# QZ1-boy/CDFO

Measured on NVIDIA B200. Metric: HR frames/sec, 1080p x4 LD-QP37, higher is better.
Workload: dtype bf16

## Files before the change

cdfo_b200/_lib.py:

```python
import ctypes
import os
import re
import weakref

import torch

_HERE = os.path.dirname(os.path.abspath(__file__))
SO_PATH = os.path.join(_HERE, "libcdfo_b200.so")

OK = 0
F32, F16, BF16 = 0, 1, 2
_DTYPES = {torch.float32: F32, torch.float16: F16, torch.bfloat16: BF16}


class CdfoError(RuntimeError):
    pass


_lib = None
HEADER = os.path.join(os.path.dirname(_HERE), "include", "cdfo_b200.h")


def _ctype(decl):
    d = decl.strip()
# ... 27 lines not shown
        fn.restype, fn.argtypes = res, args


def lib():
    global _lib
    if _lib is None:
        if not os.path.isfile(SO_PATH):
            raise CdfoError(
                "cdfo_b200: %s not found -- build it with `python cdfo_b200/csrc/build.py` "
                "(there is no CPU or PyTorch fallback for this path)" % SO_PATH)
        _lib = ctypes.CDLL(SO_PATH)
        _bind_prototypes(_lib)
    return _lib


_LAUNCHES = {"cdfo_mv_end_fix": 3, "cdfo_lra_fwd": 5, "cdfo_lra_c8_fwd": 5, "cdfo_mdta_fwd": 3, "cdfo_mdta_c8_fwd": 3, "cdfo_psnr_ssim_u8": 3,
             "cdfo_lra_mask_logits_fwd": 2,
             "cdfo_spatial_gate_c8_fwd": 2}
launch_count = 0


def call(name, *args):
    global launch_count
    rc = getattr(lib(), name)(*args)
    if rc != OK:
        check(rc, name)
    launch_count += _LAUNCHES.get(name, 1)
    return rc


def check(rc, what=""):
# ... 45 lines not shown
```

cdfo_b200/config.py:

```python
import os

tensor_core = True

dcn_gather = "tex"

conv_pair = os.environ.get("CDFO_CONV_PAIR", "1") != "0"

conv_fold_half = os.environ.get("CDFO_CONV_FOLD_HALF", "1") != "0"

conv_parity_planes = os.environ.get("CDFO_CONV_PARITY_PLANES", "1") != "0"
trunk_fused_resample = os.environ.get("CDFO_TRUNK_FUSED_RESAMPLE", "1") != "0"

head_dual = os.environ.get("CDFO_HEAD_DUAL", "1") != "0"

fused_head_dcn = os.environ.get("CDFO_FUSED_HEAD_DCN", "1") != "0"

features_c8 = os.environ.get("CDFO_FEATURES_C8", "1") != "0"
mdta_c8 = os.environ.get("CDFO_MDTA_C8", "1") != "0"
trunk_compose_1x1 = os.environ.get("CDFO_TRUNK_COMPOSE_1X1", "1") != "0"
trunk_fused_upsample = os.environ.get("CDFO_TRUNK_FUSED_UPSAMPLE", "1") != "0"
lra_logits_from_prior = os.environ.get("CDFO_LRA_LOGITS_FROM_PRIOR", "1") != "0"
```

cdfo_b200/csrc/cdfo_common.cuh:

```cuda
#pragma once
#include <cuda_bf16.h>
#include <cuda_fp16.h>
#include <cuda_runtime.h>
#include <stdarg.h>
#include <stdint.h>
#include <stdio.h>

#include "../../include/cdfo_b200.h"

namespace cdfo {

char *last_error_buf();
int fail(int code, const char *fmt, ...);

inline int check_launch(const char *what) {
  cudaError_t e = cudaGetLastError();
  if (e != cudaSuccess) return fail(CDFO_ERR_CUDA, "%s: %s", what, cudaGetErrorString(e));
  return CDFO_OK;
}

constexpr int kNumSMs = 148;

__host__ __device__ inline int ceil_div(int a, int b) { return (a + b - 1) / b; }
inline long long ceil_div_ll(long long a, long long b) { return (a + b - 1) / b; }
// ... 16 lines not shown
  const float v = __fadd_rn((float)pos, flow);
  const float g = __fsub_rn(__fdiv_rn(__fmul_rn(2.0f, v), (float)max(size - 1, 1)), 1.0f);
  return __fmul_rn(__fdiv_rn(__fadd_rn(g, 1.0f), 2.0f), (float)(size - 1));
}

struct LraTables {
  const float *kw;
  const float *kh;
  const float *k1;
  const float *r;
  float beta, bh;
};
int lra_col_sm100_launch(const float *vrow_t, const uint8_t *midx, const float *qsel, float *long_out, const LraTables &t, int B, int H, int W,
                         cudaStream_t s);

int pointwise_conv(const float *in1, const float *in2, const float *w, const float *bias, const float *resid1, const float *resid2,
                   float *out, int B, int K, int Co, int HW, int act, int mode, cudaStream_t s, void *out_c8 = nullptr,
                   int out_channels = 0, int channel0 = 0);

int conv3x3_pack_weight_raw(const float *w, void *out, int Cout, int Cin, int NT, int n_tiles, int streamed, int taps, cudaStream_t s);

}

#define CDFO_REQUIRE(cond, code, ...)                 \
  do {                                                \
    if (!(cond)) return cdfo::fail(code, __VA_ARGS__); \
  } while (0)
```

cdfo_b200/csrc/lra.cu:

```cuda
#include <cuda.h>
#include <cstring>

#include "cdfo_common.cuh"
#include "sm100_ptx.cuh"

namespace cdfo {

__device__ __forceinline__ float warp_max(float v) {
#pragma unroll
  for (int o = 16; o > 0; o >>= 1) v = fmaxf(v, __shfl_xor_sync(0xffffffffu, v, o));
  return v;
}
__device__ __forceinline__ float warp_sum(float v) {
#pragma unroll
  for (int o = 16; o > 0; o >>= 1) v += __shfl_xor_sync(0xffffffffu, v, o);
  return v;
}

__global__ void lra_mask_kernel(const float *__restrict__ u, const float *__restrict__ vmax, const float *__restrict__ qv,
                                uint8_t *__restrict__ midx, float *__restrict__ qsel, int HW) {
  __shared__ float vm[64];
  const int b = blockIdx.y;
  if (threadIdx.x < 64) vm[threadIdx.x] = vmax[b * 64 + threadIdx.x];
  __syncthreads();
// ... 836 lines not shown
  g_lra_col_tc = on != 0;
  return CDFO_OK;
}
extern "C" int cdfo_lra_set_win_tensor_core(int on) {
  g_lra_win_tc = on != 0;
  return CDFO_OK;
}

extern "C" size_t cdfo_lra_workspace_bytes(int B, int H, int W) {
  const size_t P = (size_t)B * H * W;
  return P * (1 + 4) + 3 * P * 64 * 4 + 256;
}

static int lra_run(const float *qv, const float *u, const float *vmax, const float *x, const float *x2, const float *tables,
                   float beta, float bh, const float *fuse_w, const float *fuse_b, float *out, void *out_c8, int out_channels,
                   int channel0, void *workspace, int B, int H, int W, void *stream);

extern "C" int cdfo_lra_fwd(const float *qv, const float *u, const float *vmax, const float *x, const float *x2, const float *tables,
                            float beta, float bh, const float *fuse_w, const float *fuse_b, float *out, void *workspace, int B,
                            int H, int W, void *stream) {
  return lra_run(qv, u, vmax, x, x2, tables, beta, bh, fuse_w, fuse_b, out, nullptr, 0, 0, workspace, B, H, W, stream);
}

extern "C" int cdfo_lra_c8_fwd(const float *qv, const float *u, const float *vmax, const float *x, const float *x2, const float *tables,
                               float beta, float bh, const float *fuse_w, const float *fuse_b, void *out_c8, int out_channels,
                               int channel0, void *workspace, int B, int H, int W, void *stream) {
  CDFO_REQUIRE(out_c8 && ((uintptr_t)out_c8 & 15) == 0, CDFO_ERR_NULL, "cdfo_lra_c8_fwd: out_c8 must be a 16-byte aligned pointer");
  CDFO_REQUIRE(out_channels % 8 == 0 && channel0 % 8 == 0 && channel0 >= 0 && channel0 + 64 <= out_channels, CDFO_ERR_SHAPE,
               "cdfo_lra_c8_fwd: channels [%d, %d) do not fit %d output channels (multiples of 8)", channel0, channel0 + 64, out_channels);
  return lra_run(qv, u, vmax, x, x2, tables, beta, bh, fuse_w, fuse_b, nullptr, out_c8, out_channels, channel0, workspace, B, H, W, stream);
}

static int lra_run(const float *qv, const float *u, const float *vmax, const float *x, const float *x2, const float *tables,
                   float beta, float bh, const float *fuse_w, const float *fuse_b, float *out, void *out_c8, int out_channels,
                   int channel0, void *workspace, int B, int H, int W, void *stream) {
  CDFO_REQUIRE(qv && u && vmax && x && tables && fuse_w && fuse_b && (out || out_c8) && workspace, CDFO_ERR_NULL, "cdfo_lra_fwd: NULL pointer");
  CDFO_REQUIRE(B > 0 && B <= 65535 && H > 0 && W > 0 && H % 8 == 0 && W % 8 == 0, CDFO_ERR_SHAPE,
               "cdfo_lra_fwd: H and W must be multiples of the window size 8 (got %d x %d)", H, W);
  cudaStream_t s = (cudaStream_t)stream;
  const size_t P = (size_t)B * H * W;
  const int HW = H * W;
  uint8_t *ws = (uint8_t *)workspace;
  float *qsel = (float *)ws;
  float *vrow_t = qsel + P;
  float *long_out = vrow_t + P * 64;
  float *loc_out = long_out + P * 64;
  uint8_t *midx = (uint8_t *)(loc_out + P * 64);
  LraTables t{tables, tables + 9, tables + 18, tables + 82, beta, bh};

  lra_mask_kernel<<<dim3(ceil_div(HW, 128), B), 128, 0, s>>>(u, vmax, qv, midx, qsel, HW);
// ... 42 lines not shown
  int col_done = 0;
  if (!g_lra_col_tf32 && g_lra_col_tc) {
    col_done = lra_col_sm100_launch(vrow_t, midx, qsel, long_out, t, B, H, W, s);
    if (col_done < 0) return col_done;
  }
  if (col_done) {
  } else if (g_lra_col_tf32) {
    lra_col_kernel<<<dim3(W, B), kColThreads, col_smem, s>>>(vrow_t, midx, qsel, long_out, t, H, W);
  } else {
    const size_t col16_smem = ((size_t)Hk * kQw + 64 * ((size_t)Hk / 2 + 4) + 2 * (size_t)(H + 8) + 16) * 4;
    lra_col_bf16_kernel<<<dim3(W, B), kColThreads, col16_smem, s>>>(vrow_t, midx, qsel, long_out, t, H, W);
  }
  if (g_lra_win_tc) lra_win_tc_kernel<<<dim3(W / 8, H / 8, B), kWinTcThreads, 0, s>>>(qv, midx, loc_out, H, W);
  else lra_win_kernel<<<dim3(W / 8, H / 8, B), kWinThreads, win_smem, s>>>(qv, midx, loc_out, H, W);
  if (int rc = check_launch("cdfo_lra_fwd")) return rc;
  return pointwise_conv(long_out, loc_out, fuse_w, fuse_b, x, x2, out, B, 128, 64, HW, 0, 1, s, out_c8, out_channels, channel0);
}
```

cdfo_b200/csrc/pointwise.cu:

```cuda
#include "cdfo_common.cuh"

namespace cdfo {
namespace pw {

constexpr int kTP = 64, kThreads = 256;
constexpr int kLdT = 72;

__device__ __forceinline__ uint32_t to_tf32(float x) {
  uint32_t r;
  asm("cvt.rna.tf32.f32 %0, %1;" : "=r"(r) : "f"(x));
  return r;
}
__device__ __forceinline__ void mma_tf32(float (&d)[4], const uint32_t (&a)[4], uint32_t b0, uint32_t b1) {
  asm volatile("mma.sync.aligned.m16n8k8.row.col.f32.tf32.tf32.f32 {%0, %1, %2, %3}, {%4, %5, %6, %7}, {%8, %9}, {%0, %1, %2, %3};"
               : "+f"(d[0]), "+f"(d[1]), "+f"(d[2]), "+f"(d[3])
               : "r"(a[0]), "r"(a[1]), "r"(a[2]), "r"(a[3]), "r"(b0), "r"(b1));
}

struct Params {
  const float *in1, *in2, *w, *bias, *resid1, *resid2;
  float *out;
  uint4 *out8;
  int out_chunks, chunk0;
  int HW, act;
};

__device__ __forceinline__ void cp_async16(void *dst, const void *src, bool valid) {
  const uint32_t d = (uint32_t)__cvta_generic_to_shared(dst);
  const int n = valid ? 16 : 0;
  asm volatile("cp.async.cg.shared.global [%0], [%1], 16, %2;" ::"r"(d), "l"(src), "r"(n) : "memory");
}
__device__ __forceinline__ void cp_async_commit() { asm volatile("cp.async.commit_group;" ::: "memory"); }
template <int N>
__device__ __forceinline__ void cp_async_wait() { asm volatile("cp.async.wait_group %0;" ::"n"(N) : "memory"); }
__device__ __forceinline__ uint32_t pack_bf2(float a, float b) {
  __nv_bfloat162 v = __floats2bfloat162_rn(a, b);
  return *reinterpret_cast<uint32_t *>(&v);
}

template <int K, int CO, int MODE, bool IN2>
__global__ void __launch_bounds__(kThreads, (K == 64 && CO == 128) ? 2 : 3) pointwise_kernel(const Params p) {
  constexpr int kLdW = K + 4;
  constexpr int kMT = CO / 32;
  constexpr int kIn1 = MODE == 0 ? K * kLdT : kTP * kLdW;
  constexpr int kInAll = (MODE == 0 && IN2) ? 2 * kIn1 : kIn1;
  constexpr int kBuf = kInAll > CO * kLdT ? kInAll : CO * kLdT;
  extern __shared__ __align__(16) float sm[];
  float *Wm = sm;
  float *Buf = Wm + CO * kLdW;
  const int tid = threadIdx.x, warp = tid >> 5, lane = tid & 31, g = lane >> 2, t = lane & 3;
  const int b = blockIdx.y, part = blockIdx.x, parts = gridDim.x, HW = p.HW;
  const int ntiles = (HW + kTP - 1) / kTP;
  const int t0 = (int)((long long)part * ntiles / parts), t1 = (int)((long long)(part + 1) * ntiles / parts);
  const uint32_t *Wu = reinterpret_cast<const uint32_t *>(Wm);
  const int px0 = (warp & 3) * 16, m0 = (warp >> 2) * kMT;

  auto prefetch = [&](int tile, float *dst) {
    const int p0 = tile * kTP, npx = min(kTP, HW - p0);
    if (MODE == 0) {
      const float *a = p.in1 + (size_t)b * K * HW + p0, *c = IN2 ? p.in2 + (size_t)b * K * HW + p0 : nullptr;
      for (int e = tid; e < K * (kTP / 4); e += kThreads) {
        const int k = e / (kTP / 4), q = (e % (kTP / 4)) * 4;
        const bool ok = q < npx;
        cp_async16(dst + k * kLdT + q, a + (size_t)k * HW + (ok ? q : 0), ok);
        if (IN2) cp_async16(dst + kIn1 + k * kLdT + q, c + (size_t)k * HW + (ok ? q : 0), ok);
      }
    } else {
      const float *a = p.in1 + ((size_t)b * HW + p0) * 64, *c = p.in2 + ((size_t)b * HW + p0) * 64;
      for (int e = tid; e < kTP * 32; e += kThreads) {
        const int q = e >> 5, j = e & 31;
        const bool ok = q < npx;
        cp_async16(dst + q * kLdW + j * 4, (j < 16 ? a : c) + (size_t)(ok ? q : 0) * 64 + (j & 15) * 4, ok);
      }
    }
    cp_async_commit();
  };

  if (t0 < t1) prefetch(t0, Buf);
  for (int e = tid; e < CO * K; e += kThreads) Wm[(e / K) * kLdW + (e % K)] = __uint_as_float(to_tf32(p.w[e]));

  for (int tile = t0; tile < t1; ++tile) {
    const int p0 = tile * kTP, npx = min(kTP, HW - p0);
    float *In = Buf + ((tile - t0) & 1) * kBuf;
    float *Out = In;
    if (tile + 1 < t1) {
      prefetch(tile + 1, Buf + ((tile + 1 - t0) & 1) * kBuf);
      cp_async_wait<1>();
    } else {
      cp_async_wait<0>();
    }
    __syncthreads();
    float acc[kMT][2][4];
#pragma unroll
    for (int m = 0; m < kMT; ++m)
#pragma unroll
      for (int n = 0; n < 2; ++n)
#pragma unroll
        for (int i = 0; i < 4; ++i) acc[m][n][i] = 0.f;
#pragma unroll 4
// ... 19 lines not shown
      }
    }
    __syncthreads();
#pragma unroll
    for (int m = 0; m < kMT; ++m)
#pragma unroll
      for (int n = 0; n < 2; ++n) {
        *reinterpret_cast<float2 *>(Out + ((m0 + m) * 16 + g) * kLdT + px0 + n * 8 + 2 * t) = make_float2(acc[m][n][0], acc[m][n][1]);
        *reinterpret_cast<float2 *>(Out + ((m0 + m) * 16 + g + 8) * kLdT + px0 + n * 8 + 2 * t) = make_float2(acc[m][n][2], acc[m][n][3]);
      }
    __syncthreads();
    if (p.out8) {
      for (int e = tid; e < (CO / 8) * kTP; e += kThreads) {
        const int c8 = e / kTP, q = e % kTP;
        if (q >= npx) continue;
        float v[8];
#pragma unroll
        for (int i = 0; i < 8; ++i) {
          const int co = c8 * 8 + i;
          float a = Out[co * kLdT + q] + (p.bias ? __ldg(p.bias + co) : 0.f);
          if (p.act == 1) a = fmaxf(a, 0.f);
          const size_t o = ((size_t)b * CO + co) * HW + p0 + q;
          if (p.resid1) a += __ldg(p.resid1 + o);
          if (p.resid2) a += __ldg(p.resid2 + o);
          v[i] = a;
        }
        p.out8[((size_t)b * p.out_chunks + p.chunk0 + c8) * HW + p0 + q] =
            make_uint4(pack_bf2(v[0], v[1]), pack_bf2(v[2], v[3]), pack_bf2(v[4], v[5]), pack_bf2(v[6], v[7]));
      }
    } else {
      for (int e = tid; e < CO * (kTP / 4); e += kThreads) {
        const int co = e / (kTP / 4), q = (e % (kTP / 4)) * 4;
        if (q >= npx) continue;
        float4 v = *reinterpret_cast<const float4 *>(Out + co * kLdT + q);
        const float bb = p.bias ? __ldg(p.bias + co) : 0.f;
        v.x += bb; v.y += bb; v.z += bb; v.w += bb;
        if (p.act == 1) { v.x = fmaxf(v.x, 0.f); v.y = fmaxf(v.y, 0.f); v.z = fmaxf(v.z, 0.f); v.w = fmaxf(v.w, 0.f); }
        const size_t o = ((size_t)b * CO + co) * HW + p0 + q;
        if (p.resid1) { const float4 r = __ldg(reinterpret_cast<const float4 *>(p.resid1 + o)); v.x += r.x; v.y += r.y; v.z += r.z; v.w += r.w; }
        if (p.resid2) { const float4 r = __ldg(reinterpret_cast<const float4 *>(p.resid2 + o)); v.x += r.x; v.y += r.y; v.z += r.z; v.w += r.w; }
        *reinterpret_cast<float4 *>(p.out + o) = v;
      }
    }
    __syncthreads();
  }
}

template <int K, int CO, int MODE>
__global__ void __launch_bounds__(kThreads, (K == 64 && CO == 128) ? 2 : 3) pointwise_ragged_kernel(const Params p) {
  constexpr int kLdW = K + 4;
  constexpr int kMT = CO / 32;
  extern __shared__ __align__(16) float sm[];
  float *Wm = sm;
  float *In = Wm + CO * kLdW;
  float *Out = In;
  const int tid = threadIdx.x, warp = tid >> 5, lane = tid & 31, g = lane >> 2, t = lane & 3;
  const int b = blockIdx.y, part = blockIdx.x, parts = gridDim.x, HW = p.HW;
  const int ntiles = (HW + kTP - 1) / kTP;
// ... 60 lines not shown
      }
    __syncthreads();
    for (int e = tid; e < CO * kTP; e += kThreads) {
      const int co = e / kTP, q = e % kTP;
      if (q >= npx) continue;
      float v = Out[co * kLdT + q] + (p.bias ? __ldg(p.bias + co) : 0.f);
      if (p.act == 1) v = fmaxf(v, 0.f);
      const size_t o = ((size_t)b * CO + co) * HW + p0 + q;
      if (p.resid1) v += __ldg(p.resid1 + o);
      if (p.resid2) v += __ldg(p.resid2 + o);
      p.out[o] = v;
    }
  }
}

template <int K, int CO, int MODE>
static int launch(const Params &p, int B, cudaStream_t s) {
  constexpr int kLdW = K + 4;
  constexpr int kPerSM = (K == 64 && CO == 128) ? 2 : 3;
  int parts = (kPerSM * kNumSMs) / B;
  if (parts < 1) parts = 1;
  const int ntiles = (p.HW + kTP - 1) / kTP;
  if (parts > ntiles) parts = ntiles;
  const size_t in1 = MODE == 0 ? K * kLdT : kTP * kLdW, out_f = CO * kLdT;
  if (p.HW % 4 != 0) {
    if (p.out8) return fail(CDFO_ERR_UNSUPPORTED, "cdfo_pointwise_conv_c8_fwd: H * W must be a multiple of 4");
    const size_t smem = (size_t)(CO * kLdW + (in1 > out_f ? in1 : out_f)) * 4;
    auto kern = pointwise_ragged_kernel<K, CO, MODE>;
    static bool attr = false;
    if (!attr) {
      cudaError_t e = cudaFuncSetAttribute(kern, cudaFuncAttributeMaxDynamicSharedMemorySize, (int)smem);
      if (e != cudaSuccess) return fail(CDFO_ERR_CUDA, "cudaFuncSetAttribute(pointwise): %s", cudaGetErrorString(e));
      attr = true;
    }
    kern<<<dim3(parts, B), kThreads, smem, s>>>(p);
    return check_launch("cdfo_pointwise_conv_fwd");
  }
  const bool in2 = MODE == 0 && p.in2 != nullptr;
  const size_t in_all = in2 ? 2 * in1 : in1;
  const size_t smem = (size_t)(CO * kLdW + 2 * (in_all > out_f ? in_all : out_f)) * 4;
  if (in2) {
    auto kern = pointwise_kernel<K, CO, MODE, true>;
    static bool attr = false;
    if (!attr) {
      cudaError_t e = cudaFuncSetAttribute(kern, cudaFuncAttributeMaxDynamicSharedMemorySize, (int)smem);
      if (e != cudaSuccess) return fail(CDFO_ERR_CUDA, "cudaFuncSetAttribute(pointwise): %s", cudaGetErrorString(e));
      attr = true;
    }
    kern<<<dim3(parts, B), kThreads, smem, s>>>(p);
  } else {
    auto kern = pointwise_kernel<K, CO, MODE, false>;
    static bool attr = false;
    if (!attr) {
      cudaError_t e = cudaFuncSetAttribute(kern, cudaFuncAttributeMaxDynamicSharedMemorySize, (int)smem);
      if (e != cudaSuccess) return fail(CDFO_ERR_CUDA, "cudaFuncSetAttribute(pointwise): %s", cudaGetErrorString(e));
      attr = true;
    }
    kern<<<dim3(parts, B), kThreads, smem, s>>>(p);
  }
  return check_launch("cdfo_pointwise_conv_fwd");
}

}

int pointwise_conv(const float *in1, const float *in2, const float *w, const float *bias, const float *resid1, const float *resid2,
                   float *out, int B, int K, int Co, int HW, int act, int mode, cudaStream_t s, void *out_c8, int out_channels,
                   int channel0) {
  pw::Params p{in1, in2, w, bias, resid1, resid2, out_c8 ? nullptr : out, (uint4 *)out_c8, out_channels / 8, channel0 / 8, HW, act};
  if (mode == 0 && K == 64 && Co == 64) return pw::launch<64, 64, 0>(p, B, s);
  if (mode == 0 && K == 64 && Co == 128) return pw::launch<64, 128, 0>(p, B, s);
  if (mode == 1 && K == 128 && Co == 64) return pw::launch<128, 64, 1>(p, B, s);
  return fail(CDFO_ERR_UNSUPPORTED, "cdfo_pointwise_conv_fwd: unsupported (mode %d, %d -> %d channels)", mode, K, Co);
}

}

using namespace cdfo;

extern "C" int cdfo_pointwise_conv_fwd(const float *in1, const float *in2, const float *w, const float *bias, const float *resid1,
                                       const float *resid2, float *out, int B, int K, int Co, int H, int W, int act, int mode,
                                       void *stream) {
  CDFO_REQUIRE(in1 && w && out && (mode == 0 || in2), CDFO_ERR_NULL, "cdfo_pointwise_conv_fwd: NULL pointer");
  CDFO_REQUIRE(B > 0 && B <= 65535 && H > 0 && W > 0, CDFO_ERR_SHAPE, "cdfo_pointwise_conv_fwd: bad shape");
// ... 3 lines not shown
  return pointwise_conv(in1, in2, w, bias, resid1, resid2, out, B, K, Co, H * W, act, mode, (cudaStream_t)stream, nullptr, 0, 0);
}

extern "C" int cdfo_pointwise_conv_c8_fwd(const float *in1, const float *in2, const float *w, const float *bias, const float *resid1,
                                          const float *resid2, void *out_c8, int B, int K, int Co, int H, int W, int act, int mode,
                                          int out_channels, int channel0, void *stream) {
  CDFO_REQUIRE(in1 && w && out_c8 && (mode == 0 || in2), CDFO_ERR_NULL, "cdfo_pointwise_conv_c8_fwd: NULL pointer");
  CDFO_REQUIRE(B > 0 && B <= 65535 && H > 0 && W > 0, CDFO_ERR_SHAPE, "cdfo_pointwise_conv_c8_fwd: bad shape");
  CDFO_REQUIRE(act == 0 || act == 1, CDFO_ERR_UNSUPPORTED, "cdfo_pointwise_conv_c8_fwd: act %d", act);
  CDFO_REQUIRE(out_channels % 8 == 0 && channel0 % 8 == 0 && channel0 >= 0 && channel0 + Co <= out_channels, CDFO_ERR_SHAPE,
               "cdfo_pointwise_conv_c8_fwd: channels [%d, %d) do not fit %d output channels (multiples of 8)", channel0, channel0 + Co, out_channels);
  CDFO_REQUIRE((((uintptr_t)in1 | (uintptr_t)in2 | (uintptr_t)out_c8 | (uintptr_t)resid1 | (uintptr_t)resid2) & 15) == 0, CDFO_ERR_SHAPE,
               "cdfo_pointwise_conv_c8_fwd: 16-byte alignment");
  return pointwise_conv(in1, in2, w, bias, resid1, resid2, nullptr, B, K, Co, H * W, act, mode, (cudaStream_t)stream, out_c8, out_channels, channel0);
}
```

cdfo_b200/csrc/priors.cu:

```cuda
#include "cdfo_common.cuh"

namespace cdfo {

template <typename MV>
__global__ void mv2mvs_kernel(const MV *__restrict__ mv, float *__restrict__ flows, int HW) {
  const int p = blockIdx.x * blockDim.x + threadIdx.x;
  if (p >= HW) return;
  const float a = (float)mv[p * 3 + 1];
  const float b = (float)mv[p * 3 + 0];
  const float den = __fmul_rn((float)mv[p * 3 + 2], -1.0f);
  float fx = __fdiv_rn(a, den), fy = __fdiv_rn(b, den);
  if (isnan(fx)) fx = 0.f;
  if (isnan(fy)) fy = 0.f;
  const float scale[7] = {3.0f, 2.0f, 1.0f, 0.0f, -1.0f, -2.0f, -3.0f};
#pragma unroll
  for (int f = 0; f < 7; ++f) {
    float vx, vy;
    if (f == 2) { vx = fx; vy = fy; }
    else if (f == 3) { vx = 0.f; vy = 0.f; }
    else { vx = __fmul_rn(fx, scale[f]); vy = __fmul_rn(fy, scale[f]); }
    flows[((size_t)f * 2 + 0) * HW + p] = __fdiv_rn(vx, 128.0f);
    flows[((size_t)f * 2 + 1) * HW + p] = __fdiv_rn(vy, 128.0f);
  }
}
// ... 89 lines not shown
    const float2 f = __bfloat1622float2(v[i]);
    dst[(size_t)(2 * i) * HW] = f.x;
    dst[(size_t)(2 * i + 1) * HW] = f.y;
  }
}

__global__ void __launch_bounds__(128) prior_conv_kernel(const float *__restrict__ x, const float *__restrict__ w,
                                                         const float *__restrict__ bias, float *__restrict__ y, int Co, int H, int W, int relu) {
  extern __shared__ float ws[];
  for (int e = threadIdx.x; e < Co * 9; e += blockDim.x) ws[e] = w[e];
  for (int e = threadIdx.x; e < Co; e += blockDim.x) ws[Co * 9 + e] = bias ? bias[e] : 0.f;
  __syncthreads();
  const int HW = H * W, p = blockIdx.x * blockDim.x + threadIdx.x, b = blockIdx.y;
  if (p >= HW) return;
  const int h = p / W, wq = p - h * W;
  const float *xp = x + (size_t)b * HW;
  float v[9];
#pragma unroll
  for (int i = 0; i < 3; ++i)
#pragma unroll
    for (int j = 0; j < 3; ++j) {
      const int hh = h + i - 1, ww = wq + j - 1;
      v[i * 3 + j] = (hh >= 0 && hh < H && ww >= 0 && ww < W) ? __ldg(xp + hh * W + ww) : 0.f;
    }
  float *yp = y + (size_t)b * Co * HW + p;
  for (int c = 0; c < Co; ++c) {
    float acc = ws[Co * 9 + c];
#pragma unroll
    for (int k = 0; k < 9; ++k) acc = fmaf(ws[c * 9 + k], v[k], acc);
    __stcs(yp + (size_t)c * HW, relu ? fmaxf(acc, 0.f) : acc);
  }
}

}

using namespace cdfo;

extern "C" int cdfo_prior_conv_act_fwd(const float *x, const float *w, const float *bias, float *y, int B, int Co, int H, int W, int relu,
                                       void *stream) {
  CDFO_REQUIRE(x && w && y, CDFO_ERR_NULL, "cdfo_prior_conv_fwd: NULL pointer");
  CDFO_REQUIRE(B > 0 && B <= 65535 && Co > 0 && Co <= 1024 && H > 0 && W > 0, CDFO_ERR_SHAPE, "cdfo_prior_conv_fwd: bad shape");
  prior_conv_kernel<<<dim3(ceil_div(H * W, 128), B), 128, (size_t)Co * 10 * 4, (cudaStream_t)stream>>>(x, w, bias, y, Co, H, W, relu ? 1 : 0);
  return check_launch("cdfo_prior_conv_fwd");
}
// ... 76 lines not shown
```

cdfo_b200/hotpath.py:

```python
import ctypes

import torch
import torch.nn.functional as F

from . import _lib, config, conv, dcn_sm100


def _lrelu(x):
    return F.leaky_relu(x, 0.1)


def _c(mod, x, **kw):
    return F.conv2d(x, mod.weight, mod.bias, **kw)


def _pkey(*params):
    return tuple((p.data_ptr(), str(p.device), p._version, p.dtype) for p in params)


def _module_cache(mod, slot, key, build):
    store = mod.__dict__.setdefault("_cdfo_derived", {})
    hit = store.get(slot)
    if hit is not None and hit[0] == key:
        return hit[1]
# ... 173 lines not shown
    _lib.call("cdfo_lra_mask_logits_fwd", _lib.ptr(_f32(v)), _lib.ptr(_f32(c2.weight)), _lib.ptr(_f32(c2.bias)), _lib.ptr(_f32(c3.weight).reshape(64, 64)),
              _lib.ptr(_f32(c3.bias)), _lib.ptr(vmax), _lib.ptr(ws), B, H, W, _lib.stream_ptr(v.device))
    return vmax


def _pointwise(in1, in2, weight, bias, act, mode=0, resid1=None, resid2=None):
    B, K, H, W = in1.shape
    Co = weight.size(0)
    out = torch.empty((B, Co, H, W), dtype=torch.float32, device=in1.device)
    _lib.call("cdfo_pointwise_conv_fwd", _lib.ptr(in1), _lib.ptr(in2), _lib.ptr(_f32(weight).reshape(Co, -1)), _lib.ptr(None if bias is None else _f32(bias)),
              _lib.ptr(resid1), _lib.ptr(resid2), _lib.ptr(out), B, K, Co, H, W, int(act), int(mode), _lib.stream_ptr(in1.device))
    return out


@torch.no_grad()
def long_range_attention(mod, res, x, u, x2=None, out8=None, channel0=0, res_prior=None):
    B, C, H, W = x.shape
    x = _f32(x)
    x2 = None if x2 is None else _f32(x2)
    du0 = mod.conv_du_re._modules["0"]
    if res_prior is not None:
        pc, rms1 = res_prior

        def build():
            w1 = du0.weight.detach().float().reshape(64, 64)
            return (w1 @ pc.weight.detach().float().reshape(64, 9)).contiguous(), (w1 @ pc.bias.detach().float() + du0.bias.detach().float()).contiguous()
        wv, bv = _module_cache(mod, "du0_after_prior", _pkey(du0.weight, du0.bias, pc.weight, pc.bias), build)
        rms1 = _f32(rms1)
        v = torch.empty((B, 64, H, W), dtype=torch.float32, device=x.device)
        _lib.call("cdfo_prior_conv_act_fwd", _lib.ptr(rms1), _lib.ptr(wv), _lib.ptr(bv), _lib.ptr(v), B, 64, H, W, 1, _lib.stream_ptr(x.device))
    else:
        v = _pointwise(_f32(res), None, du0.weight, du0.bias, act=1)
    vmax = mask_logits(mod, v)
    qv = _pointwise(x, x2, mod.input_conv.weight, mod.input_conv.bias, act=0)
    nbytes = _lib.lib().cdfo_lra_workspace_bytes(B, H, W)
    ws = torch.empty(nbytes, dtype=torch.uint8, device=x.device)
    tab, beta, bh = _lra_tap_tables(mod)
    if out8 is not None:
        if out8.dtype != torch.bfloat16 or not out8.is_contiguous() or out8.dim() != 5 or (out8.size(0), out8.size(2), out8.size(3), out8.size(4)) != (B, H, W, 8):
            raise _lib.CdfoError("long_range_attention: out8 must be a contiguous bf16 c8 tensor of the same batch and size")
        _lib.call("cdfo_lra_c8_fwd", _lib.ptr(qv), _lib.ptr(u.contiguous()), _lib.ptr(vmax), _lib.ptr(x), _lib.ptr(x2), _lib.ptr(tab),
                  ctypes.c_float(beta), ctypes.c_float(bh),
                  _lib.ptr(_f32(mod.fuse.weight).reshape(64, 128)), _lib.ptr(_f32(mod.fuse.bias)),
                  _lib.ptr(out8), out8.size(1) * 8, int(channel0), _lib.ptr(ws), B, H, W, _lib.stream_ptr(x.device))
        return out8
    out = torch.empty_like(x)
    _lib.call("cdfo_lra_fwd", _lib.ptr(qv), _lib.ptr(u.contiguous()), _lib.ptr(vmax), _lib.ptr(x), _lib.ptr(x2), _lib.ptr(tab),
              ctypes.c_float(beta), ctypes.c_float(bh),
              _lib.ptr(_f32(mod.fuse.weight).reshape(64, 128)), _lib.ptr(_f32(mod.fuse.bias)),
              _lib.ptr(out), _lib.ptr(ws), B, H, W, _lib.stream_ptr(x.device))
    return out


@torch.no_grad()
def prior_conv(conv_mod, x):
# ... 9 lines not shown


_SLOT = (0, 1, 2, 4, 5, 6)


@torch.no_grad()
def align_and_fuse(model, center, fea_nb, ufs_nb, rms_nb, mv_nb, u_nb, B):
    H, W = center.shape[2:]
    c8_align = (config.mdta_c8 and model.alignment == "mv_dcn" and config.dcn_gather == "tex" and config.fused_head_dcn
                and model.MV_deform_align.deformable_groups == 16)
    if c8_align:
        from . import features
        ufs_prior = features.prior_conv_c8(model.conv_expand_ufs, ufs_nb, lrelu=False)
    else:
        ufs_prior = prior_conv(model.conv_expand_ufs, ufs_nb)
    rms_prior = prior_conv(model.conv_expand_rms, rms_nb)
    runs = fea_nb if isinstance(fea_nb, (tuple, list)) else (fea_nb,)
    cat8 = torch.empty((6 * B, 16, H, W, 8), dtype=torch.bfloat16, device=center.device)
    off = 0
    for run in runs:
        sl = slice(off, off + run.size(0))
        long_range_attention(model.RDAB, rms_prior[sl], run, u_nb[sl], x2=rms_prior[sl], out8=cat8[sl], channel0=64,
                             res_prior=(model.conv_expand_rms, rms_nb[sl]) if config.lra_logits_from_prior else None)
        conv.to_c8(run, out=cat8[sl], channel0=0)
        off += run.size(0)
    fr = model.conv_expand_fea_r
    stack = torch.empty((B, 56, H, W, 8), dtype=torch.bfloat16, device=center.device)
    center8 = conv.to_c8(center)
    stack[:, 24:32] = center8
    al = model.MV_deform_align
    if c8_align:
        fea_i = conv.conv3x3(cat8, fr.weight, fr.bias, conv.ACT_NONE)
        mv_dual_att_alignment(al, center, fea_i, ufs_prior, mv_nb, stack=stack, group_chunk=[8 * f for f in _SLOT], x8=center8)
        return conv.conv3x3(stack, model.tsa_fusion.weight, model.tsa_fusion.bias, conv.ACT_LRELU)
    fea_i = conv.conv3x3(cat8, fr.weight, fr.bias, conv.ACT_NONE, out_nchw=True)
    if model.alignment == "mv_dcn" and config.dcn_gather == "tex":
        mv_dual_att_alignment(al, center, fea_i, ufs_prior, mv_nb, stack=stack, group_chunk=[8 * f for f in _SLOT])
    else:
        a8 = conv.to_c8(al(center, fea_i, ufs_prior, mv_nb)).view(6, B, 8, H, W, 8)
# ... 126 lines not shown
```

include/cdfo_b200.h:

```cpp
#ifndef CDFO_B200_H_
#define CDFO_B200_H_

#include <stddef.h>
#include <stdint.h>

#ifdef __cplusplus
extern "C" {
#endif

typedef enum cdfo_status {
  CDFO_OK = 0,
  CDFO_ERR_SHAPE = -1,
  CDFO_ERR_NULL = -2,
  CDFO_ERR_CUDA = -3,
  CDFO_ERR_UNSUPPORTED = -4,
  CDFO_ERR_NO_DEVICE = -5
} cdfo_status;

typedef enum cdfo_dtype { CDFO_F32 = 0, CDFO_F16 = 1, CDFO_BF16 = 2 } cdfo_dtype;
#define CDFO_FIELDS_F16X4 16

const char *cdfo_last_error(void);
int cdfo_version(void);
int cdfo_device_ok(int dev);
// ... 73 lines not shown
                          const float *b2, float *gate, int B, int C, int Cmid, int HW, void *stream);
int cdfo_pack_c8_scaled(const float *x_nchw, const float *scale, void *x_c8, int B, int C, int H, int W, void *stream);
int cdfo_unpack_c8_add(const void *x_c8, const float *add_nchw, int add_batch, float *y_nchw, int B, int C, int H, int W,
                       void *stream);
int cdfo_resample_c8(const void *a, const void *b, const void *base, void *y, int B, int C, int Ho, int Wo, int mode, void *stream);
int cdfo_lra_fwd(const float *qv, const float *u, const float *vmax, const float *x, const float *x2, const float *tables,
                 float beta, float bh, const float *fuse_w, const float *fuse_b, float *out, void *workspace, int B, int H, int W,
                 void *stream);
int cdfo_lra_set_col_precision(int tf32);
int cdfo_lra_set_col_tcgen05(int on);
int cdfo_lra_set_win_tensor_core(int on);
int cdfo_lra_set_row_tma(int on);
int cdfo_lra_c8_fwd(const float *qv, const float *u, const float *vmax, const float *x, const float *x2, const float *tables,
                    float beta, float bh, const float *fuse_w, const float *fuse_b, void *out_c8, int out_channels, int channel0,
                    void *workspace, int B, int H, int W, void *stream);
int cdfo_pointwise_conv_fwd(const float *in1, const float *in2, const float *w, const float *bias, const float *resid1,
                            const float *resid2, float *out, int B, int K, int Co, int H, int W, int act, int mode, void *stream);
int cdfo_pointwise_conv_c8_fwd(const float *in1, const float *in2, const float *w, const float *bias, const float *resid1,
                               const float *resid2, void *out_c8, int B, int K, int Co, int H, int W, int act, int mode,
                               int out_channels, int channel0, void *stream);
size_t cdfo_lra_workspace_bytes(int B, int H, int W);
int cdfo_layernorm_c_fwd(const void *x, const float *gamma, const float *beta, void *y, int B, int C, int H, int W, float eps,
                         int dtype, void *stream);
int cdfo_dwconv3x3_fwd(const void *x, const float *w, void *y, int B, int C, int H, int W, int dtype, void *stream);
int cdfo_mdta_gram_fwd(const void *qk, float *partial, int B, int Ctot, int H, int W, int parts, int dtype, void *stream);
int cdfo_conv3x3_pair_sm100_supported(int Cout, int Cin);
size_t cdfo_conv3x3_pair_sm100_weight_bytes(int Cout, int Cin);
int cdfo_conv3x3_pair_sm100_pack_weight(const float *w, void *wpk, int Cout, int Cin, void *stream);
int cdfo_conv3x3_pair_sm100_fwd(const void *x_c8, const void *wpk, const float *bias, const void *resid_c8, void *y_c8, int B, int Cin,
                                int Cout, int H, int W, int act, void *stream);
int cdfo_conv3x3_pair_sm100_planes_fwd(const void *x_c8, const void *wpk, const float *bias, const void *resid_c8, void *y, int B,
                                       int Cin, int Cout, int H, int W, int act, int y_planes, void *stream);
int cdfo_conv3x3_pair_sm100_edge_fwd(const void *x_c8, const void *wpk, const float *bias, const float *bias_edge, const void *resid_c8,
                                     void *y, int B, int Cin, int Cout, int H, int W, int act, int y_planes, void *stream);
int cdfo_conv3x3_pair_sm100_up2_fwd(const void *x8_1x, const void *wpk, const float *bias, const float *bias_edge, void *y, int B, int Cin,
// ... 38 lines not shown
```

Measured before the change: 90.94.

## Compute rms prior conv inside LRA pointwise kernels instead of materializing it

Removes the separate prior_conv pass that wrote a 64-channel fp32 rms prior map. The 3x3 single-channel prior convolution is recomputed from the raw rms map inside the input 1x1 conv (as in2) and inside the fuse conv epilogue (as resid2). The fuse epilogue also writes x into the c8 concat buffer, which drops the separate to_c8 copy. This saves large fp32 reads and writes and two launches, in exchange for extra per-pixel FMAs, one more shared-memory weight table, and fewer resident blocks for the prior variant (launch bounds move to 2).

```diff
diff --git a/cdfo_b200/_lib.py b/cdfo_b200/_lib.py
--- a/cdfo_b200/_lib.py
+++ b/cdfo_b200/_lib.py
@@ -65,7 +65,7 @@
     return _lib
 
 
-_LAUNCHES = {"cdfo_mv_end_fix": 3, "cdfo_lra_fwd": 5, "cdfo_lra_c8_fwd": 5, "cdfo_mdta_fwd": 3, "cdfo_mdta_c8_fwd": 3, "cdfo_psnr_ssim_u8": 3,
+_LAUNCHES = {"cdfo_mv_end_fix": 3, "cdfo_lra_fwd": 5, "cdfo_lra_c8_fwd": 5, "cdfo_lra_prior_c8_fwd": 5, "cdfo_mdta_fwd": 3, "cdfo_mdta_c8_fwd": 3, "cdfo_psnr_ssim_u8": 3,
              "cdfo_lra_mask_logits_fwd": 2,
              "cdfo_spatial_gate_c8_fwd": 2}
 launch_count = 0
diff --git a/cdfo_b200/config.py b/cdfo_b200/config.py
--- a/cdfo_b200/config.py
+++ b/cdfo_b200/config.py
@@ -20,3 +20,4 @@
 trunk_compose_1x1 = os.environ.get("CDFO_TRUNK_COMPOSE_1X1", "1") != "0"
 trunk_fused_upsample = os.environ.get("CDFO_TRUNK_FUSED_UPSAMPLE", "1") != "0"
 lra_logits_from_prior = os.environ.get("CDFO_LRA_LOGITS_FROM_PRIOR", "1") != "0"
+lra_prior_in_kernel = os.environ.get("CDFO_LRA_PRIOR_IN_KERNEL", "1") != "0"
diff --git a/cdfo_b200/csrc/cdfo_common.cuh b/cdfo_b200/csrc/cdfo_common.cuh
--- a/cdfo_b200/csrc/cdfo_common.cuh
+++ b/cdfo_b200/csrc/cdfo_common.cuh
@@ -54,9 +54,13 @@
 int lra_col_sm100_launch(const float *vrow_t, const uint8_t *midx, const float *qsel, float *long_out, const LraTables &t, int B, int H, int W,
                          cudaStream_t s);
 
+struct PwPrior {
+  const float *map, *w, *bias;
+  int H, W, x_channel0;
+};
 int pointwise_conv(const float *in1, const float *in2, const float *w, const float *bias, const float *resid1, const float *resid2,
                    float *out, int B, int K, int Co, int HW, int act, int mode, cudaStream_t s, void *out_c8 = nullptr,
-                   int out_channels = 0, int channel0 = 0);
+                   int out_channels = 0, int channel0 = 0, const PwPrior *prior = nullptr);
 
 int conv3x3_pack_weight_raw(const float *w, void *out, int Cout, int Cin, int NT, int n_tiles, int streamed, int taps, cudaStream_t s);
 
diff --git a/cdfo_b200/csrc/lra.cu b/cdfo_b200/csrc/lra.cu
--- a/cdfo_b200/csrc/lra.cu
+++ b/cdfo_b200/csrc/lra.cu
@@ -874,7 +874,7 @@
 
 static int lra_run(const float *qv, const float *u, const float *vmax, const float *x, const float *x2, const float *tables,
                    float beta, float bh, const float *fuse_w, const float *fuse_b, float *out, void *out_c8, int out_channels,
-                   int channel0, void *workspace, int B, int H, int W, void *stream);
+                   int channel0, void *workspace, int B, int H, int W, void *stream, const PwPrior *prior = nullptr);
 
 extern "C" int cdfo_lra_fwd(const float *qv, const float *u, const float *vmax, const float *x, const float *x2, const float *tables,
                             float beta, float bh, const float *fuse_w, const float *fuse_b, float *out, void *workspace, int B,
@@ -891,9 +891,25 @@
   return lra_run(qv, u, vmax, x, x2, tables, beta, bh, fuse_w, fuse_b, nullptr, out_c8, out_channels, channel0, workspace, B, H, W, stream);
 }
 
+extern "C" int cdfo_lra_prior_c8_fwd(const float *qv, const float *u, const float *vmax, const float *x, const float *prior_map,
+                                     const float *prior_w, const float *prior_b, const float *tables, float beta, float bh,
+                                     const float *fuse_w, const float *fuse_b, void *out_c8, int out_channels, int channel0, int x_channel0,
+                                     void *workspace, int B, int H, int W, void *stream) {
+  CDFO_REQUIRE(prior_map && prior_w && prior_b, CDFO_ERR_NULL, "cdfo_lra_prior_c8_fwd: NULL prior pointer");
+  CDFO_REQUIRE(out_c8 && ((uintptr_t)out_c8 & 15) == 0 && ((uintptr_t)x & 15) == 0, CDFO_ERR_NULL,
+               "cdfo_lra_prior_c8_fwd: out_c8 and x must be 16-byte aligned pointers");
+  CDFO_REQUIRE(out_channels % 8 == 0 && channel0 % 8 == 0 && channel0 >= 0 && channel0 + 64 <= out_channels && x_channel0 % 8 == 0 &&
+                   x_channel0 >= 0 && x_channel0 + 64 <= out_channels && (x_channel0 + 64 <= channel0 || channel0 + 64 <= x_channel0),
+               CDFO_ERR_SHAPE, "cdfo_lra_prior_c8_fwd: channels [%d, %d) and [%d, %d) must be disjoint multiples of 8 within %d output channels",
+               channel0, channel0 + 64, x_channel0, x_channel0 + 64, out_channels);
+  const PwPrior prior{prior_map, prior_w, prior_b, H, W, x_channel0};
+  return lra_run(qv, u, vmax, x, nullptr, tables, beta, bh, fuse_w, fuse_b, nullptr, out_c8, out_channels, channel0, workspace, B, H, W, stream,
+                 &prior);
+}
+
 static int lra_run(const float *qv, const float *u, const float *vmax, const float *x, const float *x2, const float *tables,
                    float beta, float bh, const float *fuse_w, const float *fuse_b, float *out, void *out_c8, int out_channels,
-                   int channel0, void *workspace, int B, int H, int W, void *stream) {
+                   int channel0, void *workspace, int B, int H, int W, void *stream, const PwPrior *prior) {
   CDFO_REQUIRE(qv && u && vmax && x && tables && fuse_w && fuse_b && (out || out_c8) && workspace, CDFO_ERR_NULL, "cdfo_lra_fwd: NULL pointer");
   CDFO_REQUIRE(B > 0 && B <= 65535 && H > 0 && W > 0 && H % 8 == 0 && W % 8 == 0, CDFO_ERR_SHAPE,
                "cdfo_lra_fwd: H and W must be multiples of the window size 8 (got %d x %d)", H, W);
@@ -966,5 +982,5 @@
   if (g_lra_win_tc) lra_win_tc_kernel<<<dim3(W / 8, H / 8, B), kWinTcThreads, 0, s>>>(qv, midx, loc_out, H, W);
   else lra_win_kernel<<<dim3(W / 8, H / 8, B), kWinThreads, win_smem, s>>>(qv, midx, loc_out, H, W);
   if (int rc = check_launch("cdfo_lra_fwd")) return rc;
-  return pointwise_conv(long_out, loc_out, fuse_w, fuse_b, x, x2, out, B, 128, 64, HW, 0, 1, s, out_c8, out_channels, channel0);
-}
+  return pointwise_conv(long_out, loc_out, fuse_w, fuse_b, x, x2, out, B, 128, 64, HW, 0, 1, s, out_c8, out_channels, channel0, prior);
+}
diff --git a/cdfo_b200/csrc/pointwise.cu b/cdfo_b200/csrc/pointwise.cu
--- a/cdfo_b200/csrc/pointwise.cu
+++ b/cdfo_b200/csrc/pointwise.cu
@@ -1,9 +1,11 @@
 #include "cdfo_common.cuh"
+#include "prior_tap.cuh"
 
 namespace cdfo {
 namespace pw {
 
 constexpr int kTP = 64, kThreads = 256;
+constexpr int kPwLd = 12;
 constexpr int kLdT = 72;
 
 __device__ __forceinline__ uint32_t to_tf32(float x) {
@@ -23,6 +25,8 @@
   uint4 *out8;
   int out_chunks, chunk0;
   int HW, act;
+  const float *prior_map, *prior_w, *prior_b;
+  int H, W, x_chunk0;
 };
 
 __device__ __forceinline__ void cp_async16(void *dst, const void *src, bool valid) {
@@ -38,8 +42,10 @@
   return *reinterpret_cast<uint32_t *>(&v);
 }
 
-template <int K, int CO, int MODE, bool IN2>
-__global__ void __launch_bounds__(kThreads, (K == 64 && CO == 128) ? 2 : 3) pointwise_kernel(const Params p) {
+template <int K, int CO, int MODE, bool IN2, bool PRIOR = false>
+__global__ void __launch_bounds__(kThreads, (K == 64 && CO == 128) || PRIOR ? 2 : 3) pointwise_kernel(const Params p) {
+  static_assert(!PRIOR || (MODE == 0 ? (IN2 && K == 64) : CO == 64), "the prior has 64 channels: in2 of mode 0, resid2 of mode 1");
+  static_assert(kThreads % kTP == 0, "PRIOR: each thread keeps one pixel of a tile");
   constexpr int kLdW = K + 4;
   constexpr int kMT = CO / 32;
   constexpr int kIn1 = MODE == 0 ? K * kLdT : kTP * kLdW;
@@ -48,12 +54,37 @@
   extern __shared__ __align__(16) float sm[];
   float *Wm = sm;
   float *Buf = Wm + CO * kLdW;
+  float *Pw = Buf + 2 * kBuf;
   const int tid = threadIdx.x, warp = tid >> 5, lane = tid & 31, g = lane >> 2, t = lane & 3;
   const int b = blockIdx.y, part = blockIdx.x, parts = gridDim.x, HW = p.HW;
   const int ntiles = (HW + kTP - 1) / kTP;
   const int t0 = (int)((long long)part * ntiles / parts), t1 = (int)((long long)(part + 1) * ntiles / parts);
   const uint32_t *Wu = reinterpret_cast<const uint32_t *>(Wm);
   const int px0 = (warp & 3) * 16, m0 = (warp >> 2) * kMT;
+  auto prior_taps = [&](int p0, int npx, float (&v)[9]) {
+    const int q = tid % kTP;
+    if (q < npx) {
+      const int pix = p0 + q, h = pix / p.W;
+      prior::taps(p.prior_map + (size_t)b * HW, h, pix - h * p.W, p.H, p.W, v);
+    } else {
+#pragma unroll
+      for (int i = 0; i < 9; ++i) v[i] = 0.f;
+    }
+  };
+  if (PRIOR) {
+    for (int e = tid; e < 64 * kPwLd; e += kThreads) {
+      const int k = e / kPwLd, j = e % kPwLd;
+      Pw[e] = j < 9 ? p.prior_w[k * 9 + j] : (j == 9 ? p.prior_b[k] : 0.f);
+    }
+    __syncthreads();
+  }
+
+  auto prior_at = [&](int k, const float (&v)[9]) {
+    const float4 *r = reinterpret_cast<const float4 *>(Pw + k * kPwLd);
+    const float4 a = r[0], c = r[1], d = r[2];
+    const float w[10] = {a.x, a.y, a.z, a.w, c.x, c.y, c.z, c.w, d.x, d.y};
+    return prior::channel(w, 0, w[9], v);
+  };
 
   auto prefetch = [&](int tile, float *dst) {
     const int p0 = tile * kTP, npx = min(kTP, HW - p0);
@@ -63,7 +94,7 @@
         const int k = e / (kTP / 4), q = (e % (kTP / 4)) * 4;
         const bool ok = q < npx;
         cp_async16(dst + k * kLdT + q, a + (size_t)k * HW + (ok ? q : 0), ok);
-        if (IN2) cp_async16(dst + kIn1 + k * kLdT + q, c + (size_t)k * HW + (ok ? q : 0), ok);
+        if (IN2 && !PRIOR) cp_async16(dst + kIn1 + k * kLdT + q, c + (size_t)k * HW + (ok ? q : 0), ok);
       }
     } else {
       const float *a = p.in1 + ((size_t)b * HW + p0) * 64, *c = p.in2 + ((size_t)b * HW + p0) * 64;
@@ -75,14 +106,30 @@
     }
     cp_async_commit();
   };
-
-  if (t0 < t1) prefetch(t0, Buf);
+  auto prior_fill = [&](int p0, int npx, const float (&v)[9], float *dst) {
+    const int q = tid % kTP;
+#pragma unroll
+    for (int i = 0; i < K / (kThreads / kTP); ++i) {
+      const int k = tid / kTP + i * (kThreads / kTP);
+      dst[kIn1 + k * kLdT + q] = q < npx ? prior_at(k, v) : 0.f;
+    }
+  };
+
+  float tap[9];
+  if (t0 < t1) {
+    prefetch(t0, Buf);
+    if (PRIOR && MODE == 0) {
+      prior_taps(t0 * kTP, min(kTP, HW - t0 * kTP), tap);
+      prior_fill(t0 * kTP, min(kTP, HW - t0 * kTP), tap, Buf);
+    }
+  }
   for (int e = tid; e < CO * K; e += kThreads) Wm[(e / K) * kLdW + (e % K)] = __uint_as_float(to_tf32(p.w[e]));
 
   for (int tile = t0; tile < t1; ++tile) {
     const int p0 = tile * kTP, npx = min(kTP, HW - p0);
     float *In = Buf + ((tile - t0) & 1) * kBuf;
     float *Out = In;
+    if (PRIOR) prior_taps(MODE == 0 ? p0 + kTP : p0, MODE == 0 ? min(kTP, HW - p0 - kTP) : npx, tap);
     if (tile + 1 < t1) {
       prefetch(tile + 1, Buf + ((tile + 1 - t0) & 1) * kBuf);
       cp_async_wait<1>();
@@ -132,19 +179,28 @@
       for (int e = tid; e < (CO / 8) * kTP; e += kThreads) {
         const int c8 = e / kTP, q = e % kTP;
         if (q >= npx) continue;
-        float v[8];
+        float v[8], xr[8];
 #pragma unroll
         for (int i = 0; i < 8; ++i) {
           const int co = c8 * 8 + i;
           float a = Out[co * kLdT + q] + (p.bias ? __ldg(p.bias + co) : 0.f);
           if (p.act == 1) a = fmaxf(a, 0.f);
           const size_t o = ((size_t)b * CO + co) * HW + p0 + q;
-          if (p.resid1) a += __ldg(p.resid1 + o);
-          if (p.resid2) a += __ldg(p.resid2 + o);
+          if (PRIOR) {
+            xr[i] = __ldg(p.resid1 + o);
+            a += xr[i];
+            a += prior_at(co, tap);
+          } else {
+            if (p.resid1) a += __ldg(p.resid1 + o);
+            if (p.resid2) a += __ldg(p.resid2 + o);
+          }
           v[i] = a;
         }
         p.out8[((size_t)b * p.out_chunks + p.chunk0 + c8) * HW + p0 + q] =
             make_uint4(pack_bf2(v[0], v[1]), pack_bf2(v[2], v[3]), pack_bf2(v[4], v[5]), pack_bf2(v[6], v[7]));
+        if (PRIOR)
+          p.out8[((size_t)b * p.out_chunks + p.x_chunk0 + c8) * HW + p0 + q] =
+              make_uint4(pack_bf2(xr[0], xr[1]), pack_bf2(xr[2], xr[3]), pack_bf2(xr[4], xr[5]), pack_bf2(xr[6], xr[7]));
       }
     } else {
       for (int e = tid; e < CO * (kTP / 4); e += kThreads) {
@@ -160,6 +216,7 @@
         *reinterpret_cast<float4 *>(p.out + o) = v;
       }
     }
+    if (PRIOR && MODE == 0 && tile + 1 < t1) prior_fill(p0 + kTP, min(kTP, HW - p0 - kTP), tap, Buf + ((tile + 1 - t0) & 1) * kBuf);
     __syncthreads();
   }
 }
@@ -250,6 +307,18 @@
   }
 }
 
+template <auto kern>
+static int start(const Params &p, dim3 grid, size_t smem, cudaStream_t s) {
+  static bool attr = false;
+  if (!attr) {
+    cudaError_t e = cudaFuncSetAttribute(kern, cudaFuncAttributeMaxDynamicSharedMemorySize, (int)smem);
+    if (e != cudaSuccess) return fail(CDFO_ERR_CUDA, "cudaFuncSetAttribute(pointwise): %s", cudaGetErrorString(e));
+    attr = true;
+  }
+  kern<<<grid, kThreads, smem, s>>>(p);
+  return check_launch("cdfo_pointwise_conv_fwd");
+}
+
 template <int K, int CO, int MODE>
 static int launch(const Params &p, int B, cudaStream_t s) {
   constexpr int kLdW = K + 4;
@@ -261,6 +330,7 @@
   const size_t in1 = MODE == 0 ? K * kLdT : kTP * kLdW, out_f = CO * kLdT;
   if (p.HW % 4 != 0) {
     if (p.out8) return fail(CDFO_ERR_UNSUPPORTED, "cdfo_pointwise_conv_c8_fwd: H * W must be a multiple of 4");
+    if (p.prior_map) return fail(CDFO_ERR_UNSUPPORTED, "pointwise_conv: the in-kernel prior needs H * W to be a multiple of 4");
     const size_t smem = (size_t)(CO * kLdW + (in1 > out_f ? in1 : out_f)) * 4;
     auto kern = pointwise_ragged_kernel<K, CO, MODE>;
     static bool attr = false;
@@ -272,37 +342,36 @@
     kern<<<dim3(parts, B), kThreads, smem, s>>>(p);
     return check_launch("cdfo_pointwise_conv_fwd");
   }
-  const bool in2 = MODE == 0 && p.in2 != nullptr;
+  const bool prior = p.prior_map != nullptr;
+  const bool in2 = MODE == 0 && (p.in2 != nullptr || prior);
   const size_t in_all = in2 ? 2 * in1 : in1;
-  const size_t smem = (size_t)(CO * kLdW + 2 * (in_all > out_f ? in_all : out_f)) * 4;
-  if (in2) {
-    auto kern = pointwise_kernel<K, CO, MODE, true>;
-    static bool attr = false;
-    if (!attr) {
-      cudaError_t e = cudaFuncSetAttribute(kern, cudaFuncAttributeMaxDynamicSharedMemorySize, (int)smem);
-      if (e != cudaSuccess) return fail(CDFO_ERR_CUDA, "cudaFuncSetAttribute(pointwise): %s", cudaGetErrorString(e));
-      attr = true;
-    }
-    kern<<<dim3(parts, B), kThreads, smem, s>>>(p);
-  } else {
-    auto kern = pointwise_kernel<K, CO, MODE, false>;
-    static bool attr = false;
-    if (!attr) {
-      cudaError_t e = cudaFuncSetAttribute(kern, cudaFuncAttributeMaxDynamicSharedMemorySize, (int)smem);
-      if (e != cudaSuccess) return fail(CDFO_ERR_CUDA, "cudaFuncSetAttribute(pointwise): %s", cudaGetErrorString(e));
-      attr = true;
-    }
-    kern<<<dim3(parts, B), kThreads, smem, s>>>(p);
-  }
-  return check_launch("cdfo_pointwise_conv_fwd");
+  const size_t smem = (size_t)(CO * kLdW + 2 * (in_all > out_f ? in_all : out_f) + (prior ? 64 * kPwLd : 0)) * 4;
+  const dim3 grid(parts, B);
+  if (prior) {
+    if constexpr (MODE == 1 || CO == 128) return start<pointwise_kernel<K, CO, MODE, MODE == 0, true>>(p, grid, smem, s);
+    return fail(CDFO_ERR_UNSUPPORTED, "pointwise_conv: the in-kernel prior is built for 64 -> 128 (mode 0) and 128 -> 64 (mode 1)");
+  }
+  if (in2) return start<pointwise_kernel<K, CO, MODE, true>>(p, grid, smem, s);
+  return start<pointwise_kernel<K, CO, MODE, false>>(p, grid, smem, s);
 }
 
 }
 
 int pointwise_conv(const float *in1, const float *in2, const float *w, const float *bias, const float *resid1, const float *resid2,
                    float *out, int B, int K, int Co, int HW, int act, int mode, cudaStream_t s, void *out_c8, int out_channels,
-                   int channel0) {
-  pw::Params p{in1, in2, w, bias, resid1, resid2, out_c8 ? nullptr : out, (uint4 *)out_c8, out_channels / 8, channel0 / 8, HW, act};
+                   int channel0, const PwPrior *prior) {
+  pw::Params p{in1, in2, w, bias, resid1, resid2, out_c8 ? nullptr : out, (uint4 *)out_c8, out_channels / 8, channel0 / 8, HW, act,
+               nullptr, nullptr, nullptr, 0, 0, 0};
+  if (prior) {
+    if ((mode == 0 && in2) || resid2 || !prior->map || !prior->w || !prior->bias || prior->H * prior->W != HW || (mode == 1 && !(out_c8 && resid1)))
+      return fail(CDFO_ERR_UNSUPPORTED, "pointwise_conv: in-kernel prior with a second operand, a bad size, or (mode 1) no c8 output / x");
+    p.prior_map = prior->map;
+    p.prior_w = prior->w;
+    p.prior_b = prior->bias;
+    p.H = prior->H;
+    p.W = prior->W;
+    p.x_chunk0 = prior->x_channel0 / 8;
+  }
   if (mode == 0 && K == 64 && Co == 64) return pw::launch<64, 64, 0>(p, B, s);
   if (mode == 0 && K == 64 && Co == 128) return pw::launch<64, 128, 0>(p, B, s);
   if (mode == 1 && K == 128 && Co == 64) return pw::launch<128, 64, 1>(p, B, s);
@@ -336,3 +405,13 @@
                "cdfo_pointwise_conv_c8_fwd: 16-byte alignment");
   return pointwise_conv(in1, in2, w, bias, resid1, resid2, nullptr, B, K, Co, H * W, act, mode, (cudaStream_t)stream, out_c8, out_channels, channel0);
 }
+
+extern "C" int cdfo_pointwise_conv_prior_fwd(const float *in1, const float *prior_map, const float *prior_w, const float *prior_b,
+                                             const float *w, const float *bias, float *out, int B, int H, int W, void *stream) {
+  CDFO_REQUIRE(in1 && prior_map && prior_w && prior_b && w && out, CDFO_ERR_NULL, "cdfo_pointwise_conv_prior_fwd: NULL pointer");
+  CDFO_REQUIRE(B > 0 && B <= 65535 && H > 0 && W > 0, CDFO_ERR_SHAPE, "cdfo_pointwise_conv_prior_fwd: bad shape");
+  CDFO_REQUIRE((H * W) % 4 == 0, CDFO_ERR_UNSUPPORTED, "cdfo_pointwise_conv_prior_fwd: H * W must be a multiple of 4");
+  CDFO_REQUIRE((((uintptr_t)in1 | (uintptr_t)out) & 15) == 0, CDFO_ERR_SHAPE, "cdfo_pointwise_conv_prior_fwd: 16-byte alignment");
+  const PwPrior prior{prior_map, prior_w, prior_b, H, W, 0};
+  return pointwise_conv(in1, nullptr, w, bias, nullptr, nullptr, out, B, 64, 128, H * W, 0, 0, (cudaStream_t)stream, nullptr, 0, 0, &prior);
+}
diff --git a/cdfo_b200/csrc/prior_tap.cuh b/cdfo_b200/csrc/prior_tap.cuh
--- /dev/null
+++ b/cdfo_b200/csrc/prior_tap.cuh
@@ -0,0 +1,24 @@
+#pragma once
+
+namespace cdfo {
+namespace prior {
+
+__device__ __forceinline__ void taps(const float *__restrict__ xp, int h, int w, int H, int W, float (&v)[9]) {
+#pragma unroll
+  for (int i = 0; i < 3; ++i)
+#pragma unroll
+    for (int j = 0; j < 3; ++j) {
+      const int hh = h + i - 1, ww = w + j - 1;
+      v[i * 3 + j] = (hh >= 0 && hh < H && ww >= 0 && ww < W) ? __ldg(xp + hh * W + ww) : 0.f;
+    }
+}
+
+__device__ __forceinline__ float channel(const float *w, int o, float bias, const float (&v)[9]) {
+  float acc = bias;
+#pragma unroll
+  for (int k = 0; k < 9; ++k) acc = fmaf(w[o + k], v[k], acc);
+  return acc;
+}
+
+}
+}
diff --git a/cdfo_b200/csrc/priors.cu b/cdfo_b200/csrc/priors.cu
--- a/cdfo_b200/csrc/priors.cu
+++ b/cdfo_b200/csrc/priors.cu
@@ -1,4 +1,5 @@
 #include "cdfo_common.cuh"
+#include "prior_tap.cuh"
 
 namespace cdfo {
 
@@ -127,20 +128,11 @@
   const int HW = H * W, p = blockIdx.x * blockDim.x + threadIdx.x, b = blockIdx.y;
   if (p >= HW) return;
   const int h = p / W, wq = p - h * W;
-  const float *xp = x + (size_t)b * HW;
   float v[9];
-#pragma unroll
-  for (int i = 0; i < 3; ++i)
-#pragma unroll
-    for (int j = 0; j < 3; ++j) {
-      const int hh = h + i - 1, ww = wq + j - 1;
-      v[i * 3 + j] = (hh >= 0 && hh < H && ww >= 0 && ww < W) ? __ldg(xp + hh * W + ww) : 0.f;
-    }
+  prior::taps(x + (size_t)b * HW, h, wq, H, W, v);
   float *yp = y + (size_t)b * Co * HW + p;
   for (int c = 0; c < Co; ++c) {
-    float acc = ws[Co * 9 + c];
-#pragma unroll
-    for (int k = 0; k < 9; ++k) acc = fmaf(ws[c * 9 + k], v[k], acc);
+    const float acc = prior::channel(ws, c * 9, ws[Co * 9 + c], v);
     __stcs(yp + (size_t)c * HW, relu ? fmaxf(acc, 0.f) : acc);
   }
 }
diff --git a/cdfo_b200/hotpath.py b/cdfo_b200/hotpath.py
--- a/cdfo_b200/hotpath.py
+++ b/cdfo_b200/hotpath.py
@@ -211,7 +211,9 @@
 
 
 @torch.no_grad()
-def long_range_attention(mod, res, x, u, x2=None, out8=None, channel0=0, res_prior=None):
+def long_range_attention(mod, res, x, u, x2=None, out8=None, channel0=0, res_prior=None, x_channel0=None):
+    if x_channel0 is not None and (res_prior is None or out8 is None or x2 is not None):
+        raise _lib.CdfoError("long_range_attention: x_channel0 needs res_prior and out8, and takes the place of x2")
     B, C, H, W = x.shape
     x = _f32(x)
     x2 = None if x2 is None else _f32(x2)
@@ -229,13 +231,26 @@
     else:
         v = _pointwise(_f32(res), None, du0.weight, du0.bias, act=1)
     vmax = mask_logits(mod, v)
-    qv = _pointwise(x, x2, mod.input_conv.weight, mod.input_conv.bias, act=0)
+    if x_channel0 is not None:
+        pw, pb = _f32(pc.weight), _f32(pc.bias)
+        qv = torch.empty((B, 128, H, W), dtype=torch.float32, device=x.device)
+        _lib.call("cdfo_pointwise_conv_prior_fwd", _lib.ptr(x), _lib.ptr(rms1), _lib.ptr(pw), _lib.ptr(pb),
+                  _lib.ptr(_f32(mod.input_conv.weight).reshape(128, 64)), _lib.ptr(_f32(mod.input_conv.bias)), _lib.ptr(qv), B, H, W,
+                  _lib.stream_ptr(x.device))
+    else:
+        qv = _pointwise(x, x2, mod.input_conv.weight, mod.input_conv.bias, act=0)
     nbytes = _lib.lib().cdfo_lra_workspace_bytes(B, H, W)
     ws = torch.empty(nbytes, dtype=torch.uint8, device=x.device)
     tab, beta, bh = _lra_tap_tables(mod)
     if out8 is not None:
         if out8.dtype != torch.bfloat16 or not out8.is_contiguous() or out8.dim() != 5 or (out8.size(0), out8.size(2), out8.size(3), out8.size(4)) != (B, H, W, 8):
             raise _lib.CdfoError("long_range_attention: out8 must be a contiguous bf16 c8 tensor of the same batch and size")
+        if x_channel0 is not None:
+            _lib.call("cdfo_lra_prior_c8_fwd", _lib.ptr(qv), _lib.ptr(u.contiguous()), _lib.ptr(vmax), _lib.ptr(x), _lib.ptr(rms1), _lib.ptr(pw),
+                      _lib.ptr(pb), _lib.ptr(tab), ctypes.c_float(beta), ctypes.c_float(bh),
+                      _lib.ptr(_f32(mod.fuse.weight).reshape(64, 128)), _lib.ptr(_f32(mod.fuse.bias)),
+                      _lib.ptr(out8), out8.size(1) * 8, int(channel0), int(x_channel0), _lib.ptr(ws), B, H, W, _lib.stream_ptr(x.device))
+            return out8
         _lib.call("cdfo_lra_c8_fwd", _lib.ptr(qv), _lib.ptr(u.contiguous()), _lib.ptr(vmax), _lib.ptr(x), _lib.ptr(x2), _lib.ptr(tab),
                   ctypes.c_float(beta), ctypes.c_float(bh),
                   _lib.ptr(_f32(mod.fuse.weight).reshape(64, 128)), _lib.ptr(_f32(mod.fuse.bias)),
@@ -275,15 +290,20 @@
         ufs_prior = features.prior_conv_c8(model.conv_expand_ufs, ufs_nb, lrelu=False)
     else:
         ufs_prior = prior_conv(model.conv_expand_ufs, ufs_nb)
-    rms_prior = prior_conv(model.conv_expand_rms, rms_nb)
+    prior_in_kernel = config.lra_prior_in_kernel and config.lra_logits_from_prior
+    rms_prior = None if prior_in_kernel else prior_conv(model.conv_expand_rms, rms_nb)
     runs = fea_nb if isinstance(fea_nb, (tuple, list)) else (fea_nb,)
     cat8 = torch.empty((6 * B, 16, H, W, 8), dtype=torch.bfloat16, device=center.device)
     off = 0
     for run in runs:
         sl = slice(off, off + run.size(0))
-        long_range_attention(model.RDAB, rms_prior[sl], run, u_nb[sl], x2=rms_prior[sl], out8=cat8[sl], channel0=64,
-                             res_prior=(model.conv_expand_rms, rms_nb[sl]) if config.lra_logits_from_prior else None)
-        conv.to_c8(run, out=cat8[sl], channel0=0)
+        if prior_in_kernel:
+            long_range_attention(model.RDAB, None, run, u_nb[sl], out8=cat8[sl], channel0=64, res_prior=(model.conv_expand_rms, rms_nb[sl]),
+                                 x_channel0=0)
+        else:
+            long_range_attention(model.RDAB, rms_prior[sl], run, u_nb[sl], x2=rms_prior[sl], out8=cat8[sl], channel0=64,
+                                 res_prior=(model.conv_expand_rms, rms_nb[sl]) if config.lra_logits_from_prior else None)
+            conv.to_c8(run, out=cat8[sl], channel0=0)
         off += run.size(0)
     fr = model.conv_expand_fea_r
     stack = torch.empty((B, 56, H, W, 8), dtype=torch.bfloat16, device=center.device)
diff --git a/include/cdfo_b200.h b/include/cdfo_b200.h
--- a/include/cdfo_b200.h
+++ b/include/cdfo_b200.h
@@ -111,11 +111,17 @@
 int cdfo_lra_c8_fwd(const float *qv, const float *u, const float *vmax, const float *x, const float *x2, const float *tables,
                     float beta, float bh, const float *fuse_w, const float *fuse_b, void *out_c8, int out_channels, int channel0,
                     void *workspace, int B, int H, int W, void *stream);
+int cdfo_lra_prior_c8_fwd(const float *qv, const float *u, const float *vmax, const float *x, const float *prior_map,
+                          const float *prior_w, const float *prior_b, const float *tables, float beta, float bh, const float *fuse_w,
+                          const float *fuse_b, void *out_c8, int out_channels, int channel0, int x_channel0, void *workspace, int B,
+                          int H, int W, void *stream);
 int cdfo_pointwise_conv_fwd(const float *in1, const float *in2, const float *w, const float *bias, const float *resid1,
                             const float *resid2, float *out, int B, int K, int Co, int H, int W, int act, int mode, void *stream);
 int cdfo_pointwise_conv_c8_fwd(const float *in1, const float *in2, const float *w, const float *bias, const float *resid1,
                                const float *resid2, void *out_c8, int B, int K, int Co, int H, int W, int act, int mode,
                                int out_channels, int channel0, void *stream);
+int cdfo_pointwise_conv_prior_fwd(const float *in1, const float *prior_map, const float *prior_w, const float *prior_b, const float *w,
+                                  const float *bias, float *out, int B, int H, int W, void *stream);
 size_t cdfo_lra_workspace_bytes(int B, int H, int W);
 int cdfo_layernorm_c_fwd(const void *x, const float *gamma, const float *beta, void *y, int B, int C, int H, int W, float eps,
                          int dtype, void *stream);
```

After: 91.01 (median of 6 runs). No clear change (+0.1%).
